# osmarks/meme-search-engine

Hardware: AMD Instinct MI355X
Metric: queries/sec over 1e8x1152 index @ recall@10>=0.95 (exact brute force: recall 1.0) (higher is better)
Workload: dtype f16 in, f32 accumulate, i64 fixed-point scores; 1 GPU; brute-force top-10 over 100000000 x 1152 fp16 rows, 320 queries/step, row-sharded over 1 GPU(s); rows_total=100000000, rows_per_gpu=100000000, k=10, parallelism=row-shard x1

## Files before the change

meme-search-engine_amd/csrc/scan_mfma.hip:

```cpp
#include "common.h"
#include "kernels.h"
#include <cstdlib>
#include <type_traits>

namespace mse {
namespace {

typedef _Float16 half8 __attribute__((ext_vector_type(8)));
typedef float float4v __attribute__((ext_vector_type(4)));
typedef uint32_t u32x4 __attribute__((ext_vector_type(4)));

constexpr int KB = 64;
constexpr int W = 8;
constexpr int TILE_ROWS = 32 * W;

__global__ void pack_queries_kernel(const uint16_t* __restrict__ queries, int d, int bn, uint4* __restrict__ packed) {
    const int nkb = d / KB;
    const int QT_SLOTS = bn * 8;
    const int total = nkb * QT_SLOTS;
    queries += (size_t)blockIdx.y * bn * d;
    packed += (size_t)blockIdx.y * total;
    for (int idx = blockIdx.x * blockDim.x + threadIdx.x; idx < total; idx += gridDim.x * blockDim.x) {
        const int kb = idx / QT_SLOTS;
        const int r = idx % QT_SLOTS;
        const int q = r >> 3, slot_sw = r & 7;
        const int slot = slot_sw ^ ((q >> 1) & 7);
        packed[idx] = *reinterpret_cast<const uint4*>(queries + (size_t)q * d + kb * KB + slot * 8);
    }
}

__device__ __forceinline__ half8 as_half8(const u32x4& v) { return __builtin_bit_cast(half8, v); }

template <int N> __device__ __forceinline__ void vm_wait() {
    asm volatile("s_waitcnt vmcnt(%0)" ::"n"(N) : "memory");
    __builtin_amdgcn_sched_barrier(0);
}
__device__ __forceinline__ void dma16(const void* gptr, void* lds_wave_base) {
    __builtin_amdgcn_global_load_lds((const __attribute__((address_space(1))) void*)gptr,
                                     (__attribute__((address_space(3))) void*)lds_wave_base, 16, 0, 0);
}

constexpr float MASKED_OUT = -3.402823466e+38f;
__device__ __forceinline__ uint32_t group_word(size_t group, const uint32_t* words, size_t n_words) {
    return group < n_words ? words[group] : 0u;
}

template <int S, int NCT, int ABL = 0, typename... Mask>
__global__ __launch_bounds__(W * 64) void scan_mfma_kernel(const uint16_t* __restrict__ base, size_t n_rows, int d,
                                                           const uint4* __restrict__ packed_ro,
                                                           float* __restrict__ gmax, int nq_pad, size_t n_tiles, uint32_t y_packed, uint32_t y_cols,
                                                           Mask... mask) {
    constexpr int BN = NCT * 16;
    constexpr int QT_BYTES = BN * 128;
    constexpr int QI = BN / 64;
    constexpr bool ILV = S >= 2 && !(ABL & 16);
    extern __shared__ __attribute__((aligned(16))) char smem[];
    const int tid = threadIdx.x;
    const int lane = tid & 63, wave = tid >> 6;
    const int i = lane & 15, g = lane >> 4;
    const int nkb = d / KB;
    const size_t row_bytes = (size_t)d * 2;
    const int swz = (i >> 1) & 7;
    const size_t n_groups = (n_rows + 31) / 32;
    char* const qbase = smem;
    char* const xbase = smem + 2 * QT_BYTES + wave * (S * 4096);
    gmax += (size_t)blockIdx.y * y_cols;
    const char* const packed = reinterpret_cast<const char*>(packed_ro + (size_t)blockIdx.y * y_packed) + (size_t)(wave * QI * 64 + lane) * 16;

    size_t tile = blockIdx.x;
    if (tile >= n_tiles) return;

    auto src_ptr = [&](size_t t, int u) -> const char* {
        const int r = 8 * u + (lane >> 3);
        size_t row = t * TILE_ROWS + wave * 32 + r;
        if (row >= n_rows) row = n_rows - 1;
        const int piece = (lane & 7) ^ ((r >> 1) & 7);
        return reinterpret_cast<const char*>(base) + row * row_bytes + piece * 16;
    };
    auto dma_x = [&](const char* (&rp)[4], int kblock, int stage) {
        char* dst = xbase + stage * 4096;
        if (ABL & 4) return;
#pragma unroll
        for (int u = 0; u < 4; u++) dma16(rp[u] + (size_t)kblock * 128, dst + u * 1024);
    };
    auto dma_q = [&](int kblock, int qb) {
        const char* src = packed + (size_t)kblock * QT_BYTES;
        char* dst = qbase + qb * QT_BYTES + wave * (QI * 1024);
        if (ABL & 2) return;
#pragma unroll
        for (int u = 0; u < QI; u++) dma16(src + u * 1024, dst + u * 1024);
    };

    const char* rp[4];
    const char* rn[4];
#pragma unroll
    for (int u = 0; u < 4; u++) rp[u] = src_ptr(tile, u);
    dma_q(0, 0);
#pragma unroll
    for (int j = 0; j < S - 1; j++) dma_x(rp, j % nkb, j);
    vm_wait<0>();
    __builtin_amdgcn_s_barrier();

    int buf = 0;
    while (true) {
        float4v acc[2][NCT];
#pragma unroll
        for (int rt = 0; rt < 2; rt++)
#pragma unroll
            for (int ct = 0; ct < NCT; ct++)
#pragma unroll
                for (int r = 0; r < 4; r++) acc[rt][ct][r] = 0.0f;

        const size_t next_tile = tile + gridDim.x;
        const bool has_next_tile = next_tile < n_tiles;
#pragma unroll
        for (int u = 0; u < 4; u++) rn[u] = has_next_tile ? src_ptr(next_tile, u) : rp[u];

        for (int kb0 = 0; kb0 < nkb; kb0 += S) {
#pragma unroll
            for (int j = 0; j < S; j++) {
                const int kb = kb0 + j;
                const int kq = kb + 1 == nkb ? 0 : kb + 1;
                const int kf = kb + S - 1;
                const bool x_next = kf >= nkb;
                const size_t xoff = (size_t)(kf >= nkb ? kf - nkb : kf) * 128;
                char* const xdst = xbase + ((j + S - 1) % S) * 4096;
                const char* const qsrc = packed + (size_t)kq * QT_BYTES;
                char* const qdst = qbase + (buf ^ 1) * QT_BYTES + wave * (QI * 1024);
                auto issue_piece = [&](int p) {
                    if (p < QI) { if (!(ABL & 2)) dma16(qsrc + p * 1024, qdst + p * 1024); }
                    else if (!(ABL & 4)) dma16((x_next ? rn[p - QI] : rp[p - QI]) + xoff, xdst + (p - QI) * 1024);
                };
                if (!ILV) {
#pragma unroll
                    for (int p = 0; p < QI + 4; p++) issue_piece(p);
                    vm_wait<(QI + 4) * (S - 1)>();
                } else if (S == 2) {
                    vm_wait<0>();
                }

                const u32x4* xs = reinterpret_cast<const u32x4*>(xbase + j * 4096) + i * 8;
                const u32x4* qt = reinterpret_cast<const u32x4*>(qbase + buf * QT_BYTES) + i * 8;
                const int slot_a = g ^ swz, slot_b = (4 + g) ^ swz;
                u32x4 bq[2][2];
                bq[0][0] = qt[0 * 128 + slot_a];
                bq[0][1] = qt[1 * 128 + slot_a];
                const half8 a00 = as_half8(xs[slot_a]), a10 = as_half8(xs[128 + slot_a]);
                const half8 a01 = as_half8(xs[slot_b]), a11 = as_half8(xs[128 + slot_b]);
                constexpr int NCP = NCT / 2;
#pragma unroll
                for (int t = 0; t < 2 * NCP; t++) {
                    const int ks = t / NCP, cp = t % NCP;
                    if (t + 1 < 2 * NCP) {
                        const int ks2 = (t + 1) / NCP, cp2 = (t + 1) % NCP;
                        if (!(ABL & 8)) {
                            bq[(t + 1) & 1][0] = qt[(cp2 * 2) * 128 + (ks2 ? slot_b : slot_a)];
                            bq[(t + 1) & 1][1] = qt[(cp2 * 2 + 1) * 128 + (ks2 ? slot_b : slot_a)];
                        } else {
                            bq[(t + 1) & 1][0] = bq[t & 1][1];
                            bq[(t + 1) & 1][1] = bq[t & 1][0];
                        }
                    }
                    __builtin_amdgcn_sched_barrier(0);
                    if (ILV) {
                        constexpr int STEP = (2 * NCP) / (QI + 4);
                        if (t >= 1 && (t - 1) % STEP == 0 && (t - 1) / STEP < QI + 4) {
                            issue_piece((t - 1) / STEP);
                            __builtin_amdgcn_sched_barrier(0);
                        }
                    }
                    const half8 a0 = ks ? a01 : a00;
                    const half8 a1 = ks ? a11 : a10;
#pragma unroll
                    for (int e = 0; e < 2; e++) {
                        const half8 b = as_half8(bq[t & 1][e]);
                        const int ct = cp * 2 + e;
                        if (!(ABL & 1)) {
                            acc[0][ct] = __builtin_amdgcn_mfma_f32_16x16x32_f16(a0, b, acc[0][ct], 0, 0, 0);
                            acc[1][ct] = __builtin_amdgcn_mfma_f32_16x16x32_f16(a1, b, acc[1][ct], 0, 0, 0);
                        } else {
                            asm volatile("" ::"v"(b), "v"(a0), "v"(a1));
                        }
                    }
                }
                vm_wait<4>();
                __builtin_amdgcn_s_barrier();
                buf ^= 1;
            }
        }

        const size_t group = tile * W + wave;
        if constexpr (sizeof...(Mask) != 0) {
            const uint32_t w = group_word(group, mask...) >> (4 * g);
#pragma unroll
            for (int rt = 0; rt < 2; rt++)
#pragma unroll
                for (int r = 0; r < 4; r++) {
                    if ((w >> (16 * rt + r)) & 1u) continue;
#pragma unroll
                    for (int ct = 0; ct < NCT; ct++) acc[rt][ct][r] = MASKED_OUT;
                }
        }
#pragma unroll
        for (int ct = 0; ct < NCT; ct++) {
            float m = fmaxf(fmaxf(acc[0][ct][0], acc[0][ct][1]), fmaxf(acc[0][ct][2], acc[0][ct][3]));
            m = fmaxf(m, fmaxf(fmaxf(acc[1][ct][0], acc[1][ct][1]), fmaxf(acc[1][ct][2], acc[1][ct][3])));
            m = fmaxf(m, __shfl_xor(m, 16));
            m = fmaxf(m, __shfl_xor(m, 32));
            if (g == 0 && group < n_groups) gmax[group * (size_t)nq_pad + ct * 16 + i] = m;
        }

        if (!has_next_tile) break;
        tile = next_tile;
#pragma unroll
        for (int u = 0; u < 4; u++) rp[u] = rn[u];
    }
    vm_wait<0>();
}


typedef float float16v __attribute__((ext_vector_type(16)));

#ifdef MSE_DEV_KERNELS
__device__ unsigned long long g_scan_prof[4];
__device__ __forceinline__ uint32_t memtime() { return (uint32_t)__builtin_amdgcn_s_memtime(); }
#endif

template <int S, int MF, int PROF = 0, typename... Mask>
__global__ __launch_bounds__(W * 64) void scan_mfma2d_kernel(const uint16_t* __restrict__ base, size_t n_rows, int d,
                                                             const uint4* __restrict__ packed_ro,
                                                             float* __restrict__ gmax, int nq_pad, size_t n_tiles, uint32_t y_packed, uint32_t y_cols,
                                                             Mask... mask) {
    static_assert(sizeof...(Mask) == 0 || (MF == 16 && PROF == 0), "the masked form is the product kernel's");
    constexpr int BN = 256;
    constexpr int QT_BYTES = BN * 128;
    constexpr int QI = BN / 64;
    constexpr int RG_BYTES = 64 * 128;
    extern __shared__ __attribute__((aligned(16))) char smem[];
    const int tid = threadIdx.x;
    const int lane = tid & 63, wave = tid >> 6;
    const int rg = wave >> 1, qh = wave & 1;
    const int nkb = d / KB;
    const size_t row_bytes = (size_t)d * 2;
    const size_t n_groups = (n_rows + 31) / 32;
    char* const qbase = smem;
    char* const xbase = smem + 2 * QT_BYTES + rg * (S * RG_BYTES);
    gmax += (size_t)blockIdx.y * y_cols;
    const char* const packed = reinterpret_cast<const char*>(packed_ro + (size_t)blockIdx.y * y_packed) + (size_t)(wave * QI * 64 + lane) * 16;

    size_t tile = blockIdx.x;
    if (tile >= n_tiles) return;

    auto src_ptr = [&](size_t t, int u) -> const char* {
        const int r = qh * 32 + 8 * u + (lane >> 3);
        size_t row = t * TILE_ROWS + rg * 64 + r;
        if (row >= n_rows) row = n_rows - 1;
        const int piece = (lane & 7) ^ ((r >> 1) & 7);
        return reinterpret_cast<const char*>(base) + row * row_bytes + piece * 16;
    };
    const char* rp[4];
    const char* rn[4];
#pragma unroll
    for (int u = 0; u < 4; u++) rp[u] = src_ptr(tile, u);
    {
        char* qdst = qbase + wave * (QI * 1024);
#pragma unroll
        for (int u = 0; u < QI; u++) dma16(packed + u * 1024, qdst + u * 1024);
#pragma unroll
        for (int j = 0; j < S - 1; j++)
#pragma unroll
            for (int u = 0; u < 4; u++) dma16(rp[u] + (size_t)(j % nkb) * 128, xbase + j * RG_BYTES + (qh * 4 + u) * 1024);
    }
    vm_wait<0>();
    __builtin_amdgcn_s_barrier();

    const int i = MF == 16 ? (lane & 15) : (lane & 31);
    const int g = MF == 16 ? (lane >> 4) : (lane >> 5);
    const int swz = (i >> 1) & 7;
    constexpr int NKS = MF == 16 ? 2 : 4;
    constexpr int NRT = 64 / MF, NCTW = 128 / MF;
    constexpr int NACC = MF == 16 ? 4 : 16;
    typedef typename std::conditional<MF == 16, float4v, float16v>::type accv;

    int buf = 0;
#ifdef MSE_DEV_KERNELS
    uint32_t pt_issue = 0, pt_wait = 0, pt_bar = 0, pt_n = 0, pt_last = 0;
    if constexpr (PROF == 1) pt_last = memtime();
#endif
    while (true) {
        accv acc[NRT][NCTW];
#pragma unroll
        for (int rt = 0; rt < NRT; rt++)
#pragma unroll
            for (int ct = 0; ct < NCTW; ct++)
#pragma unroll
                for (int r = 0; r < NACC; r++) acc[rt][ct][r] = 0.0f;

        const size_t next_tile = tile + gridDim.x;
        const bool has_next_tile = next_tile < n_tiles;
#pragma unroll
        for (int u = 0; u < 4; u++) rn[u] = has_next_tile ? src_ptr(next_tile, u) : rp[u];

        for (int kb0 = 0; kb0 < nkb; kb0 += S) {
#pragma unroll
            for (int j = 0; j < S; j++) {
                const int kb = kb0 + j;
                const int kq = kb + 1 == nkb ? 0 : kb + 1;
                const int kf = kb + S - 1;
                const bool x_next = kf >= nkb;
                const size_t xoff = (size_t)(kf >= nkb ? kf - nkb : kf) * 128;
                char* const xdst = xbase + ((j + S - 1) % S) * RG_BYTES + qh * 4096;
                const char* const qsrc = packed + (size_t)kq * QT_BYTES;
                char* const qdst = qbase + (buf ^ 1) * QT_BYTES + wave * (QI * 1024);
                auto issue_piece = [&](int p) {
                    if (p < QI) dma16(qsrc + p * 1024, qdst + p * 1024);
                    else dma16((x_next ? rn[p - QI] : rp[p - QI]) + xoff, xdst + (p - QI) * 1024);
                };
                if (S == 2) vm_wait<0>();

                const u32x4* xs = reinterpret_cast<const u32x4*>(xbase + j * RG_BYTES) + i * 8;
                const u32x4* qt = reinterpret_cast<const u32x4*>(qbase + buf * QT_BYTES) + (qh * 128 + i) * 8;
                auto slot = [&](int ks) { return (MF == 16 ? (4 * ks + g) : (2 * ks + g)) ^ swz; };
                half8 a[2][NRT];
#pragma unroll
                for (int rt = 0; rt < NRT; rt++) a[0][rt] = as_half8(xs[rt * (MF * 8) + slot(0)]);
                constexpr int NT = NKS * NCTW;
                u32x4 bq[3];
                bq[0] = qt[0 * (MF * 8) + slot(0)];
                bq[1] = qt[1 * (MF * 8) + slot(0)];
#pragma unroll
                for (int t = 0; t < NT; t++) {
                    const int ks = t / NCTW, ct = t % NCTW;
                    if (t + 2 < NT) bq[(t + 2) % 3] = qt[((t + 2) % NCTW) * (MF * 8) + slot((t + 2) / NCTW)];
                    if (ct == NCTW - 2 && ks + 1 < NKS) {
#pragma unroll
                        for (int rt = 0; rt < NRT; rt++) a[(ks + 1) & 1][rt] = as_half8(xs[rt * (MF * 8) + slot(ks + 1)]);
                    }
                    __builtin_amdgcn_sched_barrier(0);
                    {
                        constexpr int STEP = NT / (QI + 4);
                        if (t >= 1 && (t - 1) % STEP == 0 && (t - 1) / STEP < QI + 4) {
                            issue_piece((t - 1) / STEP);
                            __builtin_amdgcn_sched_barrier(0);
                        }
                    }
                    const half8 b = as_half8(bq[t % 3]);
                    if constexpr (PROF == 3) __builtin_amdgcn_s_setprio(1);
#pragma unroll
                    for (int rt = 0; rt < NRT; rt++) {
                        if constexpr (MF == 16) acc[rt][ct] = __builtin_amdgcn_mfma_f32_16x16x32_f16(a[ks & 1][rt], b, acc[rt][ct], 0, 0, 0);
                        else acc[rt][ct] = __builtin_amdgcn_mfma_f32_32x32x16_f16(a[ks & 1][rt], b, acc[rt][ct], 0, 0, 0);
                    }
                    if constexpr (PROF == 3) __builtin_amdgcn_s_setprio(0);
                }
#ifdef MSE_DEV_KERNELS
                if constexpr (PROF == 1) {
                    const uint32_t t0 = memtime();
                    vm_wait<4>();
                    const uint32_t t1 = memtime();
                    __builtin_amdgcn_s_barrier();
                    const uint32_t t2 = memtime();
                    pt_issue += t0 - pt_last; pt_wait += t1 - t0; pt_bar += t2 - t1; pt_n++; pt_last = t2;
                } else
#endif
                {
                    vm_wait<4>();
#ifdef MSE_DEV_KERNELS
                    if constexpr (PROF != 2)
#endif
                    __builtin_amdgcn_s_barrier();
                }
                buf ^= 1;
            }
        }

        if constexpr (sizeof...(Mask) != 0) {
#pragma unroll
            for (int p = 0; p < 2; p++) {
                const uint32_t w = group_word(tile * W + rg * 2 + p, mask...) >> (4 * g);
#pragma unroll
                for (int h = 0; h < 2; h++)
#pragma unroll
                    for (int r = 0; r < 4; r++) {
                        if ((w >> (16 * h + r)) & 1u) continue;
#pragma unroll
                        for (int ct = 0; ct < NCTW; ct++) acc[2 * p + h][ct][r] = MASKED_OUT;
                    }
            }
        }
#pragma unroll
        for (int p = 0; p < 2; p++) {
            const size_t group = tile * W + rg * 2 + p;
#pragma unroll
            for (int ct = 0; ct < NCTW; ct++) {
                float m;
                if constexpr (MF == 16) {
                    m = fmaxf(fmaxf(acc[2 * p][ct][0], acc[2 * p][ct][1]), fmaxf(acc[2 * p][ct][2], acc[2 * p][ct][3]));
                    m = fmaxf(m, fmaxf(fmaxf(acc[2 * p + 1][ct][0], acc[2 * p + 1][ct][1]), fmaxf(acc[2 * p + 1][ct][2], acc[2 * p + 1][ct][3])));
                    m = fmaxf(m, __shfl_xor(m, 16));
                    m = fmaxf(m, __shfl_xor(m, 32));
                } else {
                    m = acc[p][ct][0];
#pragma unroll
                    for (int r = 1; r < 16; r++) m = fmaxf(m, acc[p][ct][r]);
                    m = fmaxf(m, __shfl_xor(m, 32));
                }
                if (g == 0 && group < n_groups) gmax[group * (size_t)nq_pad + qh * 128 + ct * MF + i] = m;
            }
        }

        if (!has_next_tile) break;
        tile = next_tile;
#pragma unroll
        for (int u = 0; u < 4; u++) rp[u] = rn[u];
#ifdef MSE_DEV_KERNELS
        if constexpr (PROF == 1) pt_last = memtime();
#endif
    }
    vm_wait<0>();
#ifdef MSE_DEV_KERNELS
    if constexpr (PROF == 1) {
        if (lane == 0) {
            atomicAdd(&g_scan_prof[0], (unsigned long long)pt_issue); atomicAdd(&g_scan_prof[1], (unsigned long long)pt_wait);
            atomicAdd(&g_scan_prof[2], (unsigned long long)pt_bar); atomicAdd(&g_scan_prof[3], (unsigned long long)pt_n);
        }
    }
#endif
}


#ifdef MSE_DEV_KERNELS

template <int S>
__global__ __launch_bounds__(W * 64) void scan_mfma2s_kernel(const uint16_t* __restrict__ base, size_t n_rows, int d,
                                                             const uint4* __restrict__ packed_ro,
                                                             float* __restrict__ gmax, int nq_pad, size_t n_tiles, uint32_t y_packed, uint32_t y_cols) {
    static_assert(S == 3, "the specialised schedule is written for the 3-stage ring");
    constexpr int BN = 256;
    constexpr int QT_BYTES = BN * 128;
    constexpr int RG_BYTES = 64 * 128;
    constexpr int NP = 8;
    extern __shared__ __attribute__((aligned(16))) char smem[];
    const int tid = threadIdx.x;
    const int lane = tid & 63;
    const int wave = __builtin_amdgcn_readfirstlane(tid >> 6);
    const int rg = wave >> 1, qh = wave & 1;
    const bool row_wave = wave < 4;
    const int w4 = wave & 3;
    const int nkb = d / KB;
    const size_t row_bytes = (size_t)d * 2;
    char* const qbase = smem;
    char* const xring = smem + 2 * QT_BYTES;
    char* const xbase = xring + rg * (S * RG_BYTES);
    char* const xfill = xring + w4 * (S * RG_BYTES);
    char* const qfill = qbase + w4 * (NP * 1024);
    gmax += (size_t)blockIdx.y * y_cols;
    const char* const packed = reinterpret_cast<const char*>(packed_ro + (size_t)blockIdx.y * y_packed) + (size_t)w4 * (NP * 1024) + lane * 16;

    size_t tile = blockIdx.x;
    if (tile >= n_tiles) return;

    const size_t lane_off = (size_t)(lane >> 3) * row_bytes + (size_t)(((lane & 7) ^ (lane >> 4)) * 16);
    const char* const rows0 = reinterpret_cast<const char*>(base) + (size_t)w4 * 64 * row_bytes;
    auto tile_ptr = [&](size_t t) { return rows0 + t * TILE_ROWS * row_bytes + lane_off; };
    const char* lp = tile_ptr(tile);
    const char* ln = lp;
    const size_t piece_rows = 8 * row_bytes;
    auto dma_row_piece = [&](const char* p, int u, size_t koff, char* dst) {
        const char* q = (u & 1) ? reinterpret_cast<const char*>(reinterpret_cast<uintptr_t>(p) ^ 64u) : p;
        dma16(q + (u * piece_rows + koff), dst + u * 1024);
    };
    if (row_wave) {
#pragma unroll
        for (int j = 0; j < S - 1; j++)
#pragma unroll
            for (int u = 0; u < NP; u++) dma_row_piece(lp, u, (size_t)(j % nkb) * 128, xfill + j * RG_BYTES);
    } else {
#pragma unroll
        for (int u = 0; u < NP; u++) dma16(packed + u * 1024, qfill + u * 1024);
    }
    vm_wait<0>();
    __builtin_amdgcn_s_barrier();

    const int i = lane & 15, g = lane >> 4;
    const int swz = (i >> 1) & 7;
    int buf = 0;
    while (true) {
        float4v acc[4][8];
#pragma unroll
        for (int rt = 0; rt < 4; rt++)
#pragma unroll
            for (int ct = 0; ct < 8; ct++)
#pragma unroll
                for (int r = 0; r < 4; r++) acc[rt][ct][r] = 0.0f;

        const size_t next_tile = tile + gridDim.x;
        const bool has_next_tile = next_tile < n_tiles;
        ln = has_next_tile ? tile_ptr(next_tile) : lp;

        for (int kb0 = 0; kb0 < nkb; kb0 += S) {
#pragma unroll
            for (int j = 0; j < S; j++) {
                const int kb = kb0 + j;
                const int kq = kb + 1 == nkb ? 0 : kb + 1;
                const int kf = kb + S - 1;
                const char* const xp = kf >= nkb ? ln : lp;
                const size_t xoff = (size_t)(kf >= nkb ? kf - nkb : kf) * 128;
                char* const xdst = xfill + ((j + S - 1) % S) * RG_BYTES;
                const char* const qsrc = packed + (size_t)kq * QT_BYTES;
                char* const qdst = qfill + (buf ^ 1) * QT_BYTES;
                auto issue_piece = [&](int p) {
                    if (row_wave) dma_row_piece(xp, p, xoff, xdst);
                    else dma16(qsrc + p * 1024, qdst + p * 1024);
                };

                const u32x4* xs = reinterpret_cast<const u32x4*>(xbase + j * RG_BYTES) + i * 8;
                const u32x4* qt = reinterpret_cast<const u32x4*>(qbase + buf * QT_BYTES) + (qh * 128 + i) * 8;
                auto slot = [&](int ks) { return (4 * ks + g) ^ swz; };
                half8 a[2][4];
#pragma unroll
                for (int rt = 0; rt < 4; rt++) a[0][rt] = as_half8(xs[rt * 128 + slot(0)]);
                u32x4 bq[3];
                bq[0] = qt[0 * 128 + slot(0)];
                bq[1] = qt[1 * 128 + slot(0)];
#pragma unroll
                for (int t = 0; t < 16; t++) {
                    const int ks = t / 8, ct = t % 8;
                    if (t + 2 < 16) bq[(t + 2) % 3] = qt[((t + 2) % 8) * 128 + slot((t + 2) / 8)];
                    if (ct == 6 && ks == 0) {
#pragma unroll
                        for (int rt = 0; rt < 4; rt++) a[1][rt] = as_half8(xs[rt * 128 + slot(1)]);
                    }
                    __builtin_amdgcn_sched_barrier(0);
                    if (t >= 1 && (t - 1) % 2 == 0 && (t - 1) / 2 < NP) {
                        issue_piece((t - 1) / 2);
                        __builtin_amdgcn_sched_barrier(0);
                    }
                    const half8 b = as_half8(bq[t % 3]);
#pragma unroll
                    for (int rt = 0; rt < 4; rt++) acc[rt][ct] = __builtin_amdgcn_mfma_f32_16x16x32_f16(a[ks][rt], b, acc[rt][ct], 0, 0, 0);
                }
                if (row_wave) vm_wait<NP>(); else vm_wait<0>();
                __builtin_amdgcn_s_barrier();
                buf ^= 1;
            }
        }

#pragma unroll
        for (int p = 0; p < 2; p++) {
            const size_t group = tile * W + rg * 2 + p;
#pragma unroll
            for (int ct = 0; ct < 8; ct++) {
                float m = fmaxf(fmaxf(acc[2 * p][ct][0], acc[2 * p][ct][1]), fmaxf(acc[2 * p][ct][2], acc[2 * p][ct][3]));
                m = fmaxf(m, fmaxf(fmaxf(acc[2 * p + 1][ct][0], acc[2 * p + 1][ct][1]), fmaxf(acc[2 * p + 1][ct][2], acc[2 * p + 1][ct][3])));
                m = fmaxf(m, __shfl_xor(m, 16));
                m = fmaxf(m, __shfl_xor(m, 32));
                if (g == 0) gmax[group * (size_t)nq_pad + qh * 128 + ct * 16 + i] = m;
            }
        }
        if (!has_next_tile) break;
        tile = next_tile;
        lp = ln;
    }
    vm_wait<0>();
}
#endif

thread_local unsigned g_pass_count = 1;
thread_local uint32_t g_pass_packed = 0, g_pass_cols = 0;

template <typename K, typename... Mask>
int launch_kernel(K kernel, size_t lds, size_t grid, hipStream_t stream, const uint16_t* base, size_t n_rows, int d,
                  const uint4* packed, float* group_max, int nq_pad, Mask... mask) {
    const size_t n_tiles = (n_rows + TILE_ROWS - 1) / TILE_ROWS;
    if (grid > n_tiles) grid = n_tiles;
    MSE_DYN_LDS(kernel, lds);
    hipLaunchKernelGGL(kernel, dim3((unsigned)grid, g_pass_count), dim3(W * 64), lds, stream, base, n_rows, d, packed, group_max, nq_pad, n_tiles,
                       g_pass_packed, g_pass_cols, mask...);
    MSE_HIP_TRY(hipGetLastError());
    return 0;
}

template <int S, int NCT, int ABL, typename... Mask>
int launch_variant(size_t grid, hipStream_t stream, const uint16_t* base, size_t n_rows, int d, const uint4* packed,
                   float* group_max, int nq_pad, Mask... mask) {
    const size_t lds = 2 * (size_t)(NCT * 16 * 128) + (size_t)W * S * 4096;
    return launch_kernel(scan_mfma_kernel<S, NCT, ABL, Mask...>, lds, grid, stream, base, n_rows, d, packed, group_max, nq_pad, mask...);
}

#ifdef MSE_DEV_KERNELS

template <int S>
int launch_2s(size_t grid, hipStream_t stream, const uint16_t* base, size_t n_rows, int d, const uint4* packed,
              float* group_max, int nq_pad) {
    const size_t lds = 2 * (size_t)(256 * 128) + (size_t)4 * S * 8192;
    const size_t n_full = n_rows / TILE_ROWS * TILE_ROWS;
    if (n_full && launch_kernel(scan_mfma2s_kernel<S>, lds, grid, stream, base, n_full, d, packed, group_max, nq_pad)) return -1;
    if (n_full < n_rows)
        return launch_variant<S, 16, 0>(1, stream, base + n_full * (size_t)d, n_rows - n_full, d, packed,
                                        group_max + (n_full / 32) * (size_t)nq_pad, nq_pad);
    return 0;
}
#endif

template <int S, int MF, int PROF = 0, typename... Mask>
int launch_2d(size_t grid, hipStream_t stream, const uint16_t* base, size_t n_rows, int d, const uint4* packed,
              float* group_max, int nq_pad, Mask... mask) {
    const size_t lds = 2 * (size_t)(256 * 128) + (size_t)4 * S * 8192;
    return launch_kernel(scan_mfma2d_kernel<S, MF, PROF, Mask...>, lds, grid, stream, base, n_rows, d, packed, group_max, nq_pad, mask...);
}

}

int mfma_query_tile(int d) { return (d / KB) % 2 == 0 ? 320 : 256; }
int mfma_pad(int nq, int d) {
    if (nq <= 128) return 128;
    if (nq <= 192 && (d / KB) % 3 == 0) return 192;
    if (nq <= 256 || (d / KB) % 2 != 0) return 256;
    return 320;
}

size_t mfma_packed_bytes(int d) { return (size_t)(d / KB) * 320 * 128; }

int launch_scan_mfma(const uint16_t* base, size_t n_rows, int d, const uint16_t* queries_dev, int nq_pad,
                     void* packed_scratch, float* group_max, int n_cu, hipStream_t stream, hipEvent_t ev_begin,
                     hipEvent_t ev_end, int gm_stride, int n_pass, const uint32_t* mask, size_t mask_words) {
    if (n_rows == 0) return 0;
    if (n_pass < 1 || n_pass > 65535) return fail("scan_mfma: 1..65535 passes per launch");
    if (n_pass > 1 && !gm_stride) return fail("scan_mfma: batched passes need a common group-maximum stride");
    const int gs = gm_stride ? gm_stride : nq_pad;
    if (gs < nq_pad) return fail("scan_mfma: group-maximum stride below the pass width");
    if (d % 64 != 0 || d <= 0 || d > D_MAX) return fail("vector width must be a positive multiple of 64");
    if (nq_pad != 128 && nq_pad != 256 && !(nq_pad == 192 && (d / KB) % 3 == 0) && !(nq_pad == 320 && (d / KB) % 2 == 0))
        return fail("scan_mfma: query tile must be padded to 128, 192 (K blocks divisible by 3), 256 or 320 (K blocks even)");
    uint4* packed = reinterpret_cast<uint4*>(packed_scratch);
    hipLaunchKernelGGL(pack_queries_kernel, dim3(64, (unsigned)n_pass), dim3(256), 0, stream, queries_dev, d, nq_pad, packed);
    struct PassScope {
        PassScope(unsigned n, uint32_t pk, uint32_t cols) { g_pass_count = n; g_pass_packed = pk; g_pass_cols = cols; }
        ~PassScope() { g_pass_count = 1; g_pass_packed = 0; g_pass_cols = 0; }
    } pass_scope((unsigned)n_pass, (uint32_t)((size_t)(d / KB) * nq_pad * 8), (uint32_t)nq_pad);
    if (ev_begin) MSE_HIP_TRY(hipEventRecord(ev_begin, stream));
    const int nkb = d / KB;
    const int S = nkb % 3 == 0 ? 3 : nkb % 2 == 0 ? 2 : 1;
    const size_t grid = (size_t)n_cu;
    int rc = -2;
#ifdef MSE_DEV_KERNELS
    if (!mask) {
    const int abl = getenv("MSE_SCAN_ABL") ? atoi(getenv("MSE_SCAN_ABL")) : 0;
    const int v2d = getenv("MSE_SCAN_2D") ? atoi(getenv("MSE_SCAN_2D")) : -1;
    if (nq_pad == 128 && S == 3 && abl == 16) rc = launch_variant<3, 8, 16>(grid, stream, base, n_rows, d, packed, group_max, gs);
    else if (nq_pad == 256 && S == 3 && abl) {
        switch (abl) {
            case 1: rc = launch_variant<3, 16, 1>(grid, stream, base, n_rows, d, packed, group_max, gs); break;
            case 2: rc = launch_variant<3, 16, 2>(grid, stream, base, n_rows, d, packed, group_max, gs); break;
            case 4: rc = launch_variant<3, 16, 4>(grid, stream, base, n_rows, d, packed, group_max, gs); break;
            case 6: rc = launch_variant<3, 16, 6>(grid, stream, base, n_rows, d, packed, group_max, gs); break;
            case 8: rc = launch_variant<3, 16, 8>(grid, stream, base, n_rows, d, packed, group_max, gs); break;
            case 9: rc = launch_variant<3, 16, 9>(grid, stream, base, n_rows, d, packed, group_max, gs); break;
            case 14: rc = launch_variant<3, 16, 14>(grid, stream, base, n_rows, d, packed, group_max, gs); break;
            case 16: rc = launch_variant<3, 16, 16>(grid, stream, base, n_rows, d, packed, group_max, gs); break;
            default: break;
        }
    }
    else if (nq_pad == 256 && S == 3 && v2d == 0) rc = launch_variant<3, 16, 0>(grid, stream, base, n_rows, d, packed, group_max, gs);
    else if (nq_pad == 256 && S == 3 && v2d == 161) rc = launch_2d<3, 16, 1>(grid, stream, base, n_rows, d, packed, group_max, gs);
    else if (nq_pad == 256 && S == 3 && v2d == 162) rc = launch_2d<3, 16, 2>(grid, stream, base, n_rows, d, packed, group_max, gs);
    else if (nq_pad == 256 && S == 3 && v2d == 163) rc = launch_2d<3, 16, 3>(grid, stream, base, n_rows, d, packed, group_max, gs);
    else if (nq_pad == 256 && S == 3 && v2d == 17) rc = launch_2s<3>(grid, stream, base, n_rows, d, packed, group_max, gs);
    else if (nq_pad == 256 && S == 3 && v2d == 32) rc = launch_2d<3, 32>(grid, stream, base, n_rows, d, packed, group_max, gs);
    }
    if (rc != -2) {
        if (rc) return rc;
        if (ev_end) MSE_HIP_TRY(hipEventRecord(ev_end, stream));
        return 0;
    }
#endif
    auto run = [&](auto launch) { return mask ? launch(mask, mask_words) : launch(); };
    if (nq_pad == 320) {
        rc = run([&](auto... m) { return launch_variant<2, 20, 0>(grid, stream, base, n_rows, d, packed, group_max, gs, m...); });
    } else if (nq_pad == 192) {
        rc = run([&](auto... m) { return launch_variant<3, 12, 0>(grid, stream, base, n_rows, d, packed, group_max, gs, m...); });
    } else if (nq_pad == 128) {
        if (S == 3) rc = run([&](auto... m) { return launch_variant<3, 8, 0>(grid, stream, base, n_rows, d, packed, group_max, gs, m...); });
        else if (S == 2) rc = run([&](auto... m) { return launch_variant<2, 8, 0>(grid, stream, base, n_rows, d, packed, group_max, gs, m...); });
        else rc = run([&](auto... m) { return launch_variant<1, 8, 0>(grid, stream, base, n_rows, d, packed, group_max, gs, m...); });
    } else {
        if (S == 3) rc = run([&](auto... m) { return launch_2d<3, 16>(grid, stream, base, n_rows, d, packed, group_max, gs, m...); });
        else if (S == 2) rc = run([&](auto... m) { return launch_variant<2, 16, 0>(grid, stream, base, n_rows, d, packed, group_max, gs, m...); });
        else rc = run([&](auto... m) { return launch_variant<1, 16, 0>(grid, stream, base, n_rows, d, packed, group_max, gs, m...); });
    }
    if (rc) return rc;
    if (ev_end) MSE_HIP_TRY(hipEventRecord(ev_end, stream));
    return 0;
}

}

#ifdef MSE_DEV_KERNELS
extern "C" __attribute__((visibility("default"))) int mse_dev_scan_prof(unsigned long long out[4]) {
    unsigned long long z[4] = {0, 0, 0, 0};
    if (hipMemcpyFromSymbol(out, HIP_SYMBOL(mse::g_scan_prof), sizeof(z)) != hipSuccess) return -1;
    if (hipMemcpyToSymbol(HIP_SYMBOL(mse::g_scan_prof), z, sizeof(z)) != hipSuccess) return -1;
    return 0;
}
#endif
```

Baseline: 4380 queries/s.

## Route 320-query scans to the 2D MFMA kernel with two-stage ring

Generalizes the 2D MFMA scan kernel to a templated query-tile width and uses it with 320 queries for the default 320-query path, replacing the older variant kernel. For the two-stage ring it drops the per-step full vm_wait before compute, issues the row-tile DMA pieces first and the query pieces afterwards on a new schedule, and waits to zero at the close of each step instead of leaving four loads outstanding. The aim is to keep 320 queries in one block with 16x16x32 MFMA tiles and to overlap loads with MFMA better. In exchange the LDS footprint grows and the synchronisation pattern changes, which risks a stall at the step boundary.

```diff
diff --git a/meme-search-engine_amd/csrc/scan_mfma.hip b/meme-search-engine_amd/csrc/scan_mfma.hip
--- a/meme-search-engine_amd/csrc/scan_mfma.hip
+++ b/meme-search-engine_amd/csrc/scan_mfma.hip
@@ -226,15 +226,18 @@
 __device__ __forceinline__ uint32_t memtime() { return (uint32_t)__builtin_amdgcn_s_memtime(); }
 #endif
 
-template <int S, int MF, int PROF = 0, typename... Mask>
+template <int S, int MF, int PROF = 0, int BN = 256, typename... Mask>
 __global__ __launch_bounds__(W * 64) void scan_mfma2d_kernel(const uint16_t* __restrict__ base, size_t n_rows, int d,
                                                              const uint4* __restrict__ packed_ro,
                                                              float* __restrict__ gmax, int nq_pad, size_t n_tiles, uint32_t y_packed, uint32_t y_cols,
                                                              Mask... mask) {
     static_assert(sizeof...(Mask) == 0 || (MF == 16 && PROF == 0), "the masked form is the product kernel's");
-    constexpr int BN = 256;
+    static_assert(BN == 256 || (BN == 320 && MF == 16 && S == 2), "320 queries: 16x16x32 tiles on the two-stage ring only");
+    constexpr int HALF = BN / 2;
     constexpr int QT_BYTES = BN * 128;
     constexpr int QI = BN / 64;
+    constexpr bool XF = S == 2 && PROF != 4;
+    constexpr int CLOSE = S == 2 ? 0 : 4;
     constexpr int RG_BYTES = 64 * 128;
     extern __shared__ __attribute__((aligned(16))) char smem[];
     const int tid = threadIdx.x;
@@ -278,7 +281,7 @@
     const int g = MF == 16 ? (lane >> 4) : (lane >> 5);
     const int swz = (i >> 1) & 7;
     constexpr int NKS = MF == 16 ? 2 : 4;
-    constexpr int NRT = 64 / MF, NCTW = 128 / MF;
+    constexpr int NRT = 64 / MF, NCTW = HALF / MF;
     constexpr int NACC = MF == 16 ? 4 : 16;
     typedef typename std::conditional<MF == 16, float4v, float16v>::type accv;
 
@@ -313,13 +316,13 @@
                 const char* const qsrc = packed + (size_t)kq * QT_BYTES;
                 char* const qdst = qbase + (buf ^ 1) * QT_BYTES + wave * (QI * 1024);
                 auto issue_piece = [&](int p) {
-                    if (p < QI) dma16(qsrc + p * 1024, qdst + p * 1024);
-                    else dma16((x_next ? rn[p - QI] : rp[p - QI]) + xoff, xdst + (p - QI) * 1024);
+                    const int pq = XF ? p - 4 : p, px = XF ? p : p - QI;
+                    if (XF ? p >= 4 : p < QI) dma16(qsrc + pq * 1024, qdst + pq * 1024);
+                    else dma16((x_next ? rn[px] : rp[px]) + xoff, xdst + px * 1024);
                 };
-                if (S == 2) vm_wait<0>();
 
                 const u32x4* xs = reinterpret_cast<const u32x4*>(xbase + j * RG_BYTES) + i * 8;
-                const u32x4* qt = reinterpret_cast<const u32x4*>(qbase + buf * QT_BYTES) + (qh * 128 + i) * 8;
+                const u32x4* qt = reinterpret_cast<const u32x4*>(qbase + buf * QT_BYTES) + (qh * HALF + i) * 8;
                 auto slot = [&](int ks) { return (MF == 16 ? (4 * ks + g) : (2 * ks + g)) ^ swz; };
                 half8 a[2][NRT];
 #pragma unroll
@@ -339,8 +342,13 @@
                     __builtin_amdgcn_sched_barrier(0);
                     {
                         constexpr int STEP = NT / (QI + 4);
-                        if (t >= 1 && (t - 1) % STEP == 0 && (t - 1) / STEP < QI + 4) {
-                            issue_piece((t - 1) / STEP);
+                        int pc = -1;
+                        if constexpr (S == 2 && PROF != 4 && PROF != 5 && sizeof...(Mask) == 0) {
+                            if (t >= 1 && t <= 4) pc = t - 1;
+                            else if (t >= 6 && (t - 6) % 2 == 0 && (t - 6) / 2 < QI) pc = 4 + (t - 6) / 2;
+                        } else if (t >= 1 && (t - 1) % STEP == 0 && (t - 1) / STEP < QI + 4) pc = (t - 1) / STEP;
+                        if (pc >= 0) {
+                            issue_piece(pc);
                             __builtin_amdgcn_sched_barrier(0);
                         }
                     }
@@ -356,7 +364,7 @@
 #ifdef MSE_DEV_KERNELS
                 if constexpr (PROF == 1) {
                     const uint32_t t0 = memtime();
-                    vm_wait<4>();
+                    vm_wait<CLOSE>();
                     const uint32_t t1 = memtime();
                     __builtin_amdgcn_s_barrier();
                     const uint32_t t2 = memtime();
@@ -364,7 +372,7 @@
                 } else
 #endif
                 {
-                    vm_wait<4>();
+                    vm_wait<CLOSE>();
 #ifdef MSE_DEV_KERNELS
                     if constexpr (PROF != 2)
 #endif
@@ -405,7 +413,7 @@
                     for (int r = 1; r < 16; r++) m = fmaxf(m, acc[p][ct][r]);
                     m = fmaxf(m, __shfl_xor(m, 32));
                 }
-                if (g == 0 && group < n_groups) gmax[group * (size_t)nq_pad + qh * 128 + ct * MF + i] = m;
+                if (g == 0 && group < n_groups) gmax[group * (size_t)nq_pad + qh * HALF + ct * MF + i] = m;
             }
         }
 
@@ -603,11 +611,11 @@
 }
 #endif
 
-template <int S, int MF, int PROF = 0, typename... Mask>
+template <int S, int MF, int PROF = 0, int BN = 256, typename... Mask>
 int launch_2d(size_t grid, hipStream_t stream, const uint16_t* base, size_t n_rows, int d, const uint4* packed,
               float* group_max, int nq_pad, Mask... mask) {
-    const size_t lds = 2 * (size_t)(256 * 128) + (size_t)4 * S * 8192;
-    return launch_kernel(scan_mfma2d_kernel<S, MF, PROF, Mask...>, lds, grid, stream, base, n_rows, d, packed, group_max, nq_pad, mask...);
+    const size_t lds = 2 * (size_t)(BN * 128) + (size_t)4 * S * 8192;
+    return launch_kernel(scan_mfma2d_kernel<S, MF, PROF, BN, Mask...>, lds, grid, stream, base, n_rows, d, packed, group_max, nq_pad, mask...);
 }
 
 }
@@ -662,6 +670,9 @@
             default: break;
         }
     }
+    else if (nq_pad == 320 && v2d == 0) rc = launch_variant<2, 20, 0>(grid, stream, base, n_rows, d, packed, group_max, gs);
+    else if (nq_pad == 320 && v2d == 165) rc = launch_2d<2, 16, 5, 320>(grid, stream, base, n_rows, d, packed, group_max, gs);
+    else if (nq_pad == 320 && v2d == 164) rc = launch_2d<2, 16, 4, 320>(grid, stream, base, n_rows, d, packed, group_max, gs);
     else if (nq_pad == 256 && S == 3 && v2d == 0) rc = launch_variant<3, 16, 0>(grid, stream, base, n_rows, d, packed, group_max, gs);
     else if (nq_pad == 256 && S == 3 && v2d == 161) rc = launch_2d<3, 16, 1>(grid, stream, base, n_rows, d, packed, group_max, gs);
     else if (nq_pad == 256 && S == 3 && v2d == 162) rc = launch_2d<3, 16, 2>(grid, stream, base, n_rows, d, packed, group_max, gs);
@@ -677,7 +688,7 @@
 #endif
     auto run = [&](auto launch) { return mask ? launch(mask, mask_words) : launch(); };
     if (nq_pad == 320) {
-        rc = run([&](auto... m) { return launch_variant<2, 20, 0>(grid, stream, base, n_rows, d, packed, group_max, gs, m...); });
+        rc = run([&](auto... m) { return launch_2d<2, 16, 0, 320>(grid, stream, base, n_rows, d, packed, group_max, gs, m...); });
     } else if (nq_pad == 192) {
         rc = run([&](auto... m) { return launch_variant<3, 12, 0>(grid, stream, base, n_rows, d, packed, group_max, gs, m...); });
     } else if (nq_pad == 128) {
```

Result: faster. 4518 queries/s (median of 6 runs) (+3.2%).
